# hellojialee/Improved-Body-Parts

Measured on NVIDIA H100. Metric: grouping images/sec @128x128 heatmaps, 30 persons/img, higher is better.
Workload: dtype f32 body-part maps, f32 keypoint maps; f64 coordinates/scores

## Files before the change

### improved_body_parts_b200/csrc/assemble.cuh

```cuda
#pragma once

#include "common.cuh"

namespace spg {

struct AssembleArgs {
    int n_images, image_base, use_bulk;
    double len_rate, connection_tole, min_mean_score;
    int remove_recon, min_parts;
    int refresh_len_check;
    unsigned long long *wire_flag;
    unsigned long long wire_flag_value;
    unsigned int *done_counter;
    Workspace ws;
};

constexpr int kAssembleThreads = 32;

struct alignas(16) RowRec {
    double total, maxlen;
    uint32_t mask;
    int cnt, birth, alive;
};
struct alignas(16) SlotRec {
// ... 449 lines not shown
            bulk_g2s(s_cij, ws.conn_ij + img_conn, (uint32_t)(LC * sizeof(uint32_t)), &bar);
        }
    } else {
        for (size_t i = lane; i < LC; i += 32) {
            s_cs[i] = ws.conn_score[img_conn + i];
            s_cn[i] = ws.conn_norm[img_conn + i];
            s_cij[i] = ws.conn_ij[img_conn + i];
        }
    }
    for (int k = lane; k < L; k += 32) s_cc[k] = ws.conn_count[(size_t)n * L + k];
    init_person_rows(t, ws, n, lane);
    stage_peaks(t, ws, n, lane, 32, nullptr);
    __syncwarp();
    if (a.use_bulk) mbar_wait(&bar, 0);
    const AsmResult res = assemble_limbs<false>(a, t, s_cs, s_cn, s_cij, s_cc, lane, nullptr);
    __syncthreads();
    emit_people(a, t, reinterpret_cast<double *>(smem_raw), assemble_conn_bytes(L, capP), s_out, n, img_in_call, res, lane, 32);
}

__global__ void __launch_bounds__(kAssembleThreads) assemble_kernel(AssembleArgs a) {
    extern __shared__ __align__(128) unsigned char smem_raw[];
    __shared__ uint64_t bar;
    __shared__ int s_out;
    if ((int)blockIdx.x >= a.n_images) return;
    assemble_image(a, smem_raw, bar, &s_out, a.image_base + blockIdx.x, blockIdx.x, threadIdx.x);
}

}
```

### improved_body_parts_b200/csrc/common.cuh

```cuda
#pragma once

#include <cuda_runtime.h>
#include <stdint.h>

#include <algorithm>

namespace spg {

#ifdef SPG_TRACE
constexpr int kTraceCtas = 64, kTraceSlots = 1024;
__device__ unsigned long long g_spg_trace[kTraceCtas * kTraceSlots];
__device__ __forceinline__ void trace_put(int slot, int dep, int mode) {
    if (blockIdx.x < kTraceCtas && (threadIdx.x & 31) == 0) {
        unsigned long long t;
        asm volatile("mov.u64 %0, %%clock64;" : "=l"(t) : "r"(dep) : "memory");
        unsigned long long *w = &g_spg_trace[blockIdx.x * kTraceSlots + slot];
        if (mode == 2) atomicCAS(w, 0ull, t);
        else if (mode == 3) atomicMax(w, t);
        else if (mode == 4) atomicAdd(w, (unsigned long long)(unsigned)dep);
        else *w = mode == 1 ? (unsigned long long)(unsigned)dep : t;
    }
}
#define SPG_TR(slot, dep) ::spg::trace_put((slot), (int)(dep), 0)
#define SPG_TRV(slot, v) ::spg::trace_put((slot), (int)(v), 1)
// ... 48 lines not shown
    int16_t out_from_part[kMaxOutJoints];
    double *peak_x, *peak_y;
    float *peak_score;
    uint32_t *peak_anchor;
    int32_t *peak_count;
    double *cand_prio, *cand_score;
    uint32_t *cand_ij;
    unsigned long long *cand_key;
    int32_t *cand_count;
    int32_t *surv_count;
    uint32_t *conn_ij;
    double *conn_score, *conn_norm;
    int32_t *conn_count;
    double *subset;
    int32_t *n_persons;
    double *people_xy;
    double *people_score;
    uint32_t *status;
    unsigned char *wire;
    long long wire_first;
    int wire_rows;
};

__device__ __forceinline__ uint32_t smem_u32(const void *p) { return (uint32_t)__cvta_generic_to_shared(p); }

__device__ __forceinline__ void mbar_init(uint64_t *bar, uint32_t count) {
    asm volatile("mbarrier.init.shared::cta.b64 [%0], %1;" ::"r"(smem_u32(bar)), "r"(count) : "memory");
}
__device__ __forceinline__ void fence_mbar_init() { asm volatile("fence.mbarrier_init.release.cluster;" ::: "memory"); }
__device__ __forceinline__ void fence_proxy_async() { asm volatile("fence.proxy.async.shared::cta;" ::: "memory"); }
__device__ __forceinline__ void mbar_expect_tx(uint64_t *bar, uint32_t bytes) {
    asm volatile("mbarrier.arrive.expect_tx.shared::cta.b64 _, [%0], %1;" ::"r"(smem_u32(bar)), "r"(bytes) : "memory");
}
__device__ __forceinline__ void bulk_g2s(void *dst_smem, const void *src_gmem, uint32_t bytes, uint64_t *bar) {
    asm volatile("cp.async.bulk.shared::cluster.global.mbarrier::complete_tx::bytes [%0], [%1], %2, [%3];" ::"r"(
                     smem_u32(dst_smem)),
                 "l"(src_gmem), "r"(bytes), "r"(smem_u32(bar))
                 : "memory");
}
__device__ __forceinline__ void mbar_arrive(uint64_t *bar) {
    asm volatile("mbarrier.arrive.shared::cta.b64 _, [%0];" ::"r"(smem_u32(bar)) : "memory");
}
__device__ __forceinline__ bool mbar_try_wait(uint64_t *bar, uint32_t parity) {
    uint32_t ok;
    asm volatile(
        "{\n"
// ... 50 lines not shown
```

### improved_body_parts_b200/csrc/group_unbounded.cuh

```cuda
#pragma once

#include <cub/cub.cuh>

#include "assemble.cuh"
#include "limb_score.cuh"
#include "nms_peaks.cuh"

namespace spg {

constexpr int kUbPeakThreads = 1024;
constexpr int kUbScoreThreads = 128;
constexpr int kUbAssembleThreads = 1024;
constexpr int kUbMaxPeaks = 65535;
constexpr int kUbMaxRows = 32767;

struct UbArgs {
    Workspace ws;
    const float *heat;
    const void *paf;
    int64_t heat_chan_stride, paf_chan_stride;
    int H, W;
    int32_t *row_count;
    const int64_t *row_off;
    const int64_t *seg_off;
    unsigned long long *cand_key_out;
    const uint32_t *sorted;
    uint32_t *cand_idx;
    unsigned char *used;
    PersonTable table;
};

template <bool WRITE>
__global__ void __launch_bounds__(kUbPeakThreads) ub_peaks_kernel(UbArgs u, NmsArgs a) {
    using Scan = cub::BlockScan<int, kUbPeakThreads>;
    __shared__ typename Scan::TempStorage scan_tmp;
    const int c = blockIdx.x, tid = threadIdx.x;
    const int H = u.H, W = u.W;
    const float *plane = u.heat + (int64_t)c * u.heat_chan_stride;
    const int64_t npix = (int64_t)H * W;
    int base = 0;
    for (int64_t p0 = 0; p0 < npix; p0 += kUbPeakThreads) {
        const int64_t p = p0 + tid;
        int y = 0, x = 0, pk = 0;
        if (p < npix) {
            y = (int)(p / W);
            x = (int)(p - (int64_t)y * W);
            pk = nms_is_peak(plane, 0, H, W, y, x, plane[p], a.thr) ? 1 : 0;
        }
        int pos, total;
        Scan(scan_tmp).ExclusiveSum(pk, pos, total);
        if (WRITE && pk) nms_finish_peak(a, plane, H, W, (size_t)c * u.ws.capP + base + pos, y, x);
        base += total;
        __syncthreads();
    }
    if (!WRITE && tid == 0) u.ws.peak_count[c] = base;
}

__device__ __forceinline__ unsigned long long ub_prio_key(double prio) {
    const unsigned long long b = (unsigned long long)__double_as_longlong(__dadd_rn(prio, 0.0));
    return (b >> 63) ? ~b : (b | 0x8000000000000000ull);
}

template <typename T, typename TA, bool WRITE>
__global__ void __launch_bounds__(kUbScoreThreads) ub_score_kernel(UbArgs u, ScoreArgs sa) {
    __shared__ double s_rcp[kScreenMaxMid + 1];
    for (int m = threadIdx.x; m <= kScreenMaxMid; m += blockDim.x) s_rcp[m] = m > 0 ? __ddiv_rn(1.0, (double)m) : 0.0;
    __syncthreads();
    const Workspace &ws = u.ws;
    const int k = blockIdx.x, i = blockIdx.y * kUbScoreThreads + threadIdx.x;
    const int pa = ws.limbs[2 * k], pb = ws.limbs[2 * k + 1];
    const int nA = ws.peak_count[pa], nB = ws.peak_count[pb];
    if (i >= nA || nB == 0) return;
    const int capP = ws.capP, H = u.H, W = u.W;
    const T *plane = reinterpret_cast<const T *>(u.paf) + (int64_t)k * u.paf_chan_stride;
    const PairGeom g{ws.peak_x + (size_t)pa * capP, ws.peak_y + (size_t)pa * capP, ws.peak_x + (size_t)pb * capP,
                     ws.peak_y + (size_t)pb * capP, ws.peak_score + (size_t)pa * capP, ws.peak_score + (size_t)pb * capP, s_rcp};
    const bool ain = inside_map(g.ax[i], g.ay[i], H, W);
    const TA thre2 = (TA)sa.thre2;
    const size_t slot = (size_t)k * capP + i;
    const int64_t out = WRITE ? u.row_off[slot] : 0;
    int nc = 0;
    bool bad = false;
    for (int j = 0; j < nB; j++) {
        double score, prio;
        const bool ok = score_pair_exact<T, 1, TA>(plane, H, W, sa, g, i, j, ain && inside_map(g.bx[j], g.by[j], H, W), thre2,
                                                   score, prio, bad);
        if (ok) {
            if (WRITE) {
                const int64_t o = out + nc;
                ws.cand_prio[o] = prio;
                ws.cand_score[o] = score;
                ws.cand_ij[o] = ((uint32_t)i << 16) | (uint32_t)j;
                ws.cand_key[o] = ub_prio_key(prio);
                u.cand_idx[o] = (uint32_t)o;
            }
            nc++;
        }
    }
    if (!WRITE) u.row_count[slot] = nc;
    if (bad) atomicOr(ws.status, kStSampleIndex);
}

__global__ void ub_match_kernel(UbArgs u) {
    const Workspace &ws = u.ws;
    const int k = blockIdx.x * blockDim.x + threadIdx.x;
    if (k >= ws.L) return;
    const int capP = ws.capP;
    const int pa = ws.limbs[2 * k], pb = ws.limbs[2 * k + 1];
    const int nA = ws.peak_count[pa], nB = ws.peak_count[pb];
    const int64_t c0 = u.seg_off[k], c1 = u.seg_off[k + 1];
    ws.cand_count[k] = (int)(c1 - c0);
    if (nA == 0 || nB == 0) {
        ws.conn_count[k] = -1;
        return;
    }
    unsigned char *usedA = u.used + (size_t)k * 2 * capP, *usedB = usedA + capP;
    const int lim = min(nA, nB);
    const size_t cb = (size_t)k * capP;
    int m = 0;
    for (int64_t c = c0; c < c1 && m < lim; c++) {
        const uint32_t idx = u.sorted[c];
        const uint32_t ij = ws.cand_ij[idx];
        const int i = (int)(ij >> 16), j = (int)(ij & 0xffff);
        if (usedA[i] || usedB[j]) continue;
        usedA[i] = 1;
        usedB[j] = 1;
        const double vx = __dsub_rn(ws.peak_x[(size_t)pb * capP + j], ws.peak_x[(size_t)pa * capP + i]);
        const double vy = __dsub_rn(ws.peak_y[(size_t)pb * capP + j], ws.peak_y[(size_t)pa * capP + i]);
        ws.conn_ij[cb + m] = ij;
        ws.conn_score[cb + m] = ws.cand_score[idx];
        ws.conn_norm[cb + m] = __dsqrt_rn(__dadd_rn(__dmul_rn(vx, vx), __dmul_rn(vy, vy)));
        m++;
    }
    ws.conn_count[k] = m;
}

__global__ void __launch_bounds__(kUbAssembleThreads) ub_assemble_kernel(UbArgs u, AssembleArgs a) {
    __shared__ int s_out;
    const Workspace &ws = a.ws;
    const PersonTable &t = u.table;
    const int tid = threadIdx.x, K = ws.K, L = ws.L, capP = ws.capP, capR = ws.capR;
    if (tid == 0) {
        int off = 0;
        for (int c = 0; c < K; c++) {
            t.off[c] = off;
            off += ws.peak_count[c];
        }
        t.off[K] = off;
    }
    for (int i = tid; i < K * capP; i += kUbAssembleThreads) {
        t.owner[i] = -1;
        t.ps[i] = ws.peak_score[i];
    }
    __syncthreads();
    int nrows = 0;
    if (tid == 0) {
        for (int k = 0; k < L; k++) {
            const int cc = ws.conn_count[k];
            if (cc < 0) continue;
            ConnCtx c;
// ... 41 lines not shown
```

### improved_body_parts_b200/csrc/limb_match.cuh

```cuda
#pragma once

#include "common.cuh"

namespace spg {

struct MatchArgs {
    int n_images, image_base, keys_valid;
    Workspace ws;
};

constexpr int kMatchThreads = 128;
constexpr int kMatchRegF64 = 16;
constexpr int kMatchRegCands = 16;

__device__ __forceinline__ bool key_better(double pa, int ia, double pb, int ib) {
    return pa > pb || (pa == pb && ia < ib);
}

__device__ __forceinline__ unsigned long long ordered_bits(double v) {
    const unsigned long long b = (unsigned long long)__double_as_longlong(v);
    return (b & 0x8000000000000000ull) ? ~b : (b | 0x8000000000000000ull);
}

template <int NS>
// ... 302 lines not shown
        case 5: case 6: m = match_rounds_ld<6>(sc, ws.capP, key8, nC, lane, 400 + 8 * k, ws.cand_score + cbase); break;
        default: m = match_rounds_ld<kMatchLdSlots>(sc, ws.capP, key8, nC, lane, 400 + 8 * k, ws.cand_score + cbase); break;
    }
    SPG_TR(400 + 8 * k + 5, m);
    if (coords_bar) mbar_wait(coords_bar, 0);
    for (int e = lane; e < m; e += 32) {
        const unsigned long long ke = sc.acc_key[e];
        const double score = ws.cand_score[cbase + sc.acc_cidx[e]];
        int rank = 0;
        for (int f = 0; f < m; f++) rank += sc.acc_key[f] > ke ? 1 : 0;
        const uint32_t ij = ~(uint32_t)ke;
        const int i = (int)(ij >> 16), j = (int)(ij & 0xffffu);
        const double vx = __dsub_rn(bx[j], ax[i]), vy = __dsub_rn(by[j], ay[i]);
        o_ij[rank] = ij;
        o_score[rank] = score;
        o_norm[rank] = __dsqrt_rn(__dadd_rn(__dmul_rn(vx, vx), __dmul_rn(vy, vy)));
    }
    __syncwarp();
    SPG_TR(400 + 8 * k + 6, m);
    return m;
}

__global__ void __launch_bounds__(kMatchThreads) limb_match_kernel(MatchArgs a) {
    const Workspace &ws = a.ws;
    const int lane = threadIdx.x & 31;
    const int w = (int)((blockIdx.x * (size_t)blockDim.x + threadIdx.x) >> 5);
    if (w >= a.n_images * ws.L) return;
    const int k = w % ws.L;
    const int n = a.image_base + w / ws.L;
    const size_t slot = (size_t)n * ws.L + k;
    const size_t obase = slot * ws.capP;
    const int m = match_limb(ws, n, k, lane, a.keys_valid != 0, ws.conn_ij + obase, ws.conn_score + obase, ws.conn_norm + obase);
    if (lane == 0) ws.conn_count[slot] = m;
}

}
```

### improved_body_parts_b200/csrc/limb_score.cuh

```cuda
#pragma once

#include "common.cuh"

namespace spg {

struct ScoreArgs {
    const void *paf;
    int64_t img_stride, chan_stride;
    int H, W, image_base, mid_num, screen;
    int crit1_strict;
    int exact_warps;
    double image_extent, thre2, connect_ration;
    Workspace ws;
};

constexpr int kScoreThreads = 512;
constexpr uint32_t kBulkChunkBytes = 32768;
constexpr int kScreenMaxMid = 63;
#ifndef SPG_SCREEN_SAMPLES
#define SPG_SCREEN_SAMPLES 10
#endif
constexpr int kScreenSamples = SPG_SCREEN_SAMPLES;
constexpr int kScreenMaxDim = 2048;
constexpr int kScreenSpreadFirst = kScreenSamples < 6 ? kScreenSamples : 6;
// ... 360 lines not shown
        while (lo < hi) {
            const int mid = (lo + hi + 1) >> 1;
            if ((int)s_prefix[mid] <= sidx) lo = mid; else hi = mid - 1;
        }
        const int bit = __fns(s_mask[lo], 0, sidx - (int)s_prefix[lo] + 1);
        const int p = (lo << 5) + bit;
        const int i = nB > 1 ? (int)__umulhi((uint32_t)p, magic) : p;
        const int j = p - i * nB;
        double score, prio;
        bool bad = false;
        const bool ok = score_pair_exact<T, 1, TA>(plane, H, W, a, g, i, j, s_ain[i] && s_bin[j], thre2_exact, score, prio, bad);
        if (bad) atomicOr(&s_flags, kStSampleIndex);
        if (ok) {
            const int pos = atomicAdd(&s_count, 1);
            if (pos < ws.capC) store_candidate<TA>(ws, out_base, pos, i, j, score, prio);
        }
    }
    __syncthreads();
    if (tid == 0) publish_limb(ws, n, slot, s_count, total_surv, s_flags);
}

template <typename T, bool STAGE, typename TA = T>
__global__ void __launch_bounds__(kScoreThreads, 3) limb_score_kernel(ScoreArgs a) {
    limb_score_plane<T, STAGE, TA>(a, a.ws, blockIdx.x / a.ws.L, blockIdx.x % a.ws.L);
}

struct ScoreImage {
    const void *paf;
    int64_t chan_stride;
    double image_extent;
    int H, W, slot;
};
constexpr int kScoreRaggedMaxImages = 128;
struct ScoreRagged {
    ScoreImage img[kScoreRaggedMaxImages];
};

template <typename T, bool STAGE, typename TA = T>
__global__ void __launch_bounds__(kScoreThreads, 3) limb_score_ragged_kernel(ScoreArgs a, const __grid_constant__ ScoreRagged r) {
    const ScoreImage &im = r.img[blockIdx.x / a.ws.L];
    ScoreArgs b = a;
    b.paf = im.paf;
    b.img_stride = 0;
    b.chan_stride = im.chan_stride;
    b.H = im.H;
    b.W = im.W;
    b.image_extent = im.image_extent;
    b.image_base = im.slot;
    limb_score_plane<T, STAGE, TA>(b, a.ws, 0, blockIdx.x % a.ws.L);
}

}
```

### improved_body_parts_b200/csrc/limb_score_persist.cuh

```cuda
#pragma once

#include "limb_score.cuh"

namespace spg {

constexpr int kPersistThreads = 1024;
constexpr int kPersistSlots = 3;
constexpr int kMetaSlots = 5;
constexpr int kWorkerWarps = kPersistThreads / 32 - 1;
constexpr int kPersistMaxCapP = 64;
constexpr int kScreenTailBypass = 4;
constexpr int kPersistListCap = 1024;

constexpr int kTrItemWords = 16, kTrItems = 64;
#define SPG_TR_ITEM(kind, j, f, dep) do { if ((j) < kTrItems) kind(kTrItemWords * (j) + (f), dep); } while (0)

struct PersistHdr {
    int nA, nB, npairs, n, k, special;
    uint32_t magic;
    int pad;
};

struct alignas(16) PeakSlot {
    double ax[kPersistMaxCapP], ay[kPersistMaxCapP], bx[kPersistMaxCapP], by[kPersistMaxCapP];
// ... 86 lines not shown
    const int H = a.H, W = a.W, capP = ws.capP, L = ws.L;
    const size_t plane_bytes = (size_t)H * W * sizeof(T);
    const size_t plane_stride = (plane_bytes + 127) & ~(size_t)127;
    double *s_rcp = reinterpret_cast<double *>(smem_raw);
    ScreenTab *s_tab = reinterpret_cast<ScreenTab *>(s_rcp + (kScreenMaxMid + 1));
    float *s_ts = reinterpret_cast<float *>(s_tab + (kScreenMaxMid + 1));
    MetaSlot *s_meta = reinterpret_cast<MetaSlot *>(smem_raw + screen_tables_bytes());
    unsigned char *s_planes = smem_raw + kPersistPlaneOffset;
    const int nE = min(max(a.exact_warps, 1), kWorkerWarps - 1), nS = kWorkerWarps - nE;

    if (tid == 0) {
        for (int s = 0; s < kPersistSlots; s++) {
            mbar_init(&bar_full[s], 2);
        }
        for (int e = 0; e < kMetaSlots; e++) {
            mbar_init(&bar_screened[e], nS);
            mbar_init(&bar_mfree[e], nE);
            s_meta[e].nsurv = 0; s_meta[e].ncand = 0; s_meta[e].bnext = 0; s_meta[e].flags = 0;
        }
        s_bias_bytes = 4u * kScreenBias * (uint32_t)(W + 1);
        fence_mbar_init();
    }
    if (tid >= 32 && tid < 32 + kScreenMaxMid + 1) build_screen_row(a, tid - 32, s_rcp, s_tab, s_ts, true);
    __syncthreads();

    const bool screen = a.screen && a.mid_num <= kScreenMaxMid && H <= kScreenMaxDim && W <= kScreenMaxDim;
    const T thre2 = sizeof(TA) == 8 ? f32_not_above(a.thre2) : (T)a.thre2;
    const TA thre2_exact = (TA)a.thre2;
    auto plane_of = [&](int n_local, int k) {
        return reinterpret_cast<const T *>(a.paf) + (int64_t)n_local * a.img_stride + (int64_t)k * a.chan_stride;
    };

    if (warp == 0) {
        constexpr int kMaxE = kPersistMaxCapP / 32;
        double r_xa[kMaxE], r_ya[kMaxE], r_xb[kMaxE], r_yb[kMaxE];
        float r_sa[kMaxE], r_sb[kMaxE];
        int r_cntA = 0, r_cntB = 0, r_item = 0;
        auto fetch = [&]() {
            int t = 0;
            if (lane == 0) t = (int)atomicAdd(queue, 1u);
            r_item = __shfl_sync(0xffffffffu, t, 0);
            const int item = min(r_item, n_items - 1);
            const int n_local = item / L, k = item - n_local * L;
            const int n = a.image_base + n_local;
            const int pa = ws.limbs[2 * k], pb = ws.limbs[2 * k + 1];
            r_cntA = ws.peak_count[(size_t)n * ws.K + pa];
            r_cntB = ws.peak_count[(size_t)n * ws.K + pb];
// ... 184 lines not shown
```

### improved_body_parts_b200/csrc/match_assemble.cuh

```cuda
#pragma once

#include "assemble.cuh"
#include "limb_match.cuh"

namespace spg {

constexpr int kMAMatchWarps = 7;
constexpr int kMAThreads = 32 * (1 + kMAMatchWarps);
constexpr int kMAMaxThreads = 512;

inline size_t match_assemble_smem_bytes(int K, int L, int capP, int capR, int n_match) {
    return assemble_conn_bytes(L, capP) + assemble_smem_bytes(K, capP, capR) + 2 * (size_t)K * capP * sizeof(double) +
           (size_t)n_match * match_scratch_bytes(capP);
}

__global__ void __launch_bounds__(kMAMaxThreads) match_assemble_kernel(AssembleArgs a, int keys_valid) {
    extern __shared__ __align__(128) unsigned char smem_raw[];
    __shared__ int s_ready[kMaxLimbs];
    __shared__ AsmResult s_res;
    __shared__ int s_out;
    __shared__ uint64_t s_bar;
    const Workspace &ws = a.ws;
    if ((int)blockIdx.x >= a.n_images) return;
    const int n = a.image_base + blockIdx.x;
    const int tid = threadIdx.x, lane = tid & 31, warp = tid >> 5;
    const int K = ws.K, L = ws.L, capP = ws.capP, capR = ws.capR;
    SPG_TR(warp == 0 ? 0 : 2 + warp, 0);
    const size_t LC = (size_t)L * capP;
    double *s_cs = reinterpret_cast<double *>(smem_raw);
    double *s_cn = s_cs + LC;
    uint32_t *s_cij = reinterpret_cast<uint32_t *>(s_cn + LC);
    int *s_cc = reinterpret_cast<int *>(s_cij + LC);
    unsigned char *table_base = smem_raw + assemble_conn_bytes(L, capP);
    PersonTable t = make_person_table(table_base, K, capP, capR);
    double *s_xy = reinterpret_cast<double *>(table_base + assemble_smem_bytes(K, capP, capR));
    t.px = s_xy;
    t.py = s_xy + (size_t)K * capP;
    const int n_match = (int)blockDim.x / 32 - 1;
    if (tid < L) s_ready[tid] = 0;
    const bool bulk = a.use_bulk != 0;
    if (tid == 0 && bulk) {
        mbar_init(&s_bar, 1);
        fence_mbar_init();
    }
    __syncthreads();
    if (tid == 0 && bulk) {
        const size_t KP = (size_t)K * capP, g = (size_t)n * KP;
        mbar_expect_tx(&s_bar, (uint32_t)(KP * (sizeof(float) + 2 * sizeof(double))));
        bulk_g2s(t.ps, ws.peak_score + g, (uint32_t)(KP * sizeof(float)), &s_bar);
        bulk_g2s(s_xy, ws.peak_x + g, (uint32_t)(KP * sizeof(double)), &s_bar);
        bulk_g2s(s_xy + KP, ws.peak_y + g, (uint32_t)(KP * sizeof(double)), &s_bar);
    }
    if (warp == 0) {
        SPG_TR(1, 0);
        init_person_rows(t, ws, n, lane);
        __syncwarp();
        if (bulk) mbar_wait(&s_bar, 0);
        const AsmResult res = assemble_limbs<true>(a, t, s_cs, s_cn, s_cij, s_cc, lane, s_ready);
        if (lane == 0) s_res = res;
    } else {
        if (!bulk) {
            stage_peaks(t, ws, n, tid - 32, 32 * n_match, s_xy);
            asm volatile("bar.sync 1, %0;" ::"r"(32 * n_match) : "memory");
        }
        unsigned char *scratch = reinterpret_cast<unsigned char *>(s_xy + 2 * (size_t)K * capP) + (size_t)(warp - 1) * match_scratch_bytes(capP);
        for (int k = warp - 1; k < L; k += n_match) {
            uint32_t *o_ij = s_cij + (size_t)k * capP;
// ... 28 lines not shown
```

### improved_body_parts_b200/csrc/nms_peaks.cuh

```cuda
#pragma once

#include "common.cuh"

namespace spg {

struct NmsArgs {
    const float *heat;
    int64_t img_stride, chan_stride;
    int H, W, band_rows, radius, use_bulk, image_base;
    float thr;
    Workspace ws;
};

constexpr int kNmsThreads = 256;
constexpr int kNmsBufs = 3;

__device__ __forceinline__ bool nms_is_peak(const float *buf, int lo, int H, int W, int y, int x, float v, float thr) {
    if (!(v >= thr) || v == 0.0f) return false;
#pragma unroll
    for (int dy = -1; dy <= 1; dy++) {
        const int yy = y + dy;
        if (yy < 0 || yy >= H) continue;
        const float *row = buf + (size_t)(yy - lo) * W;
#pragma unroll
// ... 162 lines not shown

    const Workspace &ws = a.ws;
    const int tid = threadIdx.x;
    const int n = a.image_base + n_local;
    const int H = a.H, W = a.W, br = a.band_rows;
    const float *plane = a.heat + (int64_t)n_local * a.img_stride + (int64_t)c * a.chan_stride;

    const int nb = (H + br - 1) / br;
    const size_t band_floats = nb == 1 ? (size_t)H * W : (size_t)(br + 2) * W;
    const size_t buf_stride = (band_floats + 31) & ~(size_t)31;
    const int nbufs = min(nb, kNmsBufs);
    float *buf0 = reinterpret_cast<float *>(smem_raw);
    uint32_t *s_list = reinterpret_cast<uint32_t *>(buf0 + (size_t)nbufs * buf_stride);
    uint32_t *s_sorted = s_list + ws.capP;
    uint16_t *s_queue = reinterpret_cast<uint16_t *>(s_sorted + ws.capP);

    if (tid == 0) {
        s_count = 0;
        if (a.use_bulk) {
            for (int i = 0; i < kNmsBufs; i++) mbar_init(&bar[i], 1);
            fence_mbar_init();
        }
    }
    __syncthreads();

    auto band_lo = [&](int b) { return max(b * br - 1, 0); };
    auto band_hi = [&](int b) { return min((b + 1) * br + 1, H); };
    auto issue = [&](int b) {
        const int lo = band_lo(b), hi = band_hi(b);
        const uint32_t bytes = (uint32_t)(hi - lo) * W * sizeof(float);
        mbar_expect_tx(&bar[b % kNmsBufs], bytes);
        bulk_g2s(buf0 + (size_t)(b % kNmsBufs) * buf_stride, plane + (size_t)lo * W, bytes, &bar[b % kNmsBufs]);
    };

    if (a.use_bulk && tid == 0)
        for (int b = 0; b < nbufs; b++) issue(b);

    for (int b = 0; b < nb; b++) {
        float *buf = a.use_bulk ? buf0 + (size_t)(b % kNmsBufs) * buf_stride : buf0;
        const int lo = band_lo(b), hi = band_hi(b);
        if (a.use_bulk) {
            mbar_wait(&bar[b % kNmsBufs], (b / kNmsBufs) & 1);
        } else {
            const int cnt = (hi - lo) * W;
            for (int i = tid; i < cnt; i += kNmsThreads) buf[i] = plane[(size_t)lo * W + i];
            __syncthreads();
// ... 99 lines not shown
```

### improved_body_parts_b200/csrc/nms_peaks_banded.cuh

```cuda
#pragma once

#include "nms_peaks_persist.cuh"

namespace spg {

constexpr int kNmsBMaxSlots = 16;
constexpr int kNmsBTeams = 4;
constexpr int kNmsBBandGroups = 1024;

struct NmsBanding {
    int band_rows, n_bands, slots, teams;
    size_t band_stride, smem;
};
inline NmsBanding nms_banding(int H, int W, int capP, size_t smem_limit) {
    NmsBanding g{};
    const int W4 = W / 4;
    const size_t fixed = kNmsPLists * (size_t)capP * sizeof(uint32_t) + (size_t)kNmsPScanners * 32 * kNmsPMaxIter * sizeof(uint16_t) + 64;
    if (smem_limit <= fixed) return g;
    g.teams = kNmsBTeams;
    const int team_warps = kNmsPScanners / kNmsBTeams;
    g.band_rows = std::max(1, std::min(H, kNmsBBandGroups / std::max(W4, 1)));
    if ((size_t)g.band_rows * W4 > (size_t)team_warps * 32 * kNmsPMaxIter) return g;
    g.n_bands = (H + g.band_rows - 1) / g.band_rows;
    g.band_stride = (((size_t)std::min(g.band_rows + 2, H) * W * sizeof(float)) + 127) & ~(size_t)127;
// ... 10 lines not shown
    const Workspace &ws = a.ws;
    const int tid = threadIdx.x, lane = tid & 31, warp = tid >> 5;
    const int H = a.H, W = a.W, K = ws.K, capP = ws.capP;
    const int BR = a.band_rows, S = n_slots, NB = n_bands;
    constexpr int T = kNmsBTeams, TW = kNmsPScanners / kNmsBTeams;
    const size_t band_stride = (((size_t)min(BR + 2, H) * W * sizeof(float)) + 127) & ~(size_t)127;
    uint32_t *s_lists = reinterpret_cast<uint32_t *>(smem_raw + (size_t)S * band_stride);
    uint16_t *s_queues = reinterpret_cast<uint16_t *>(s_lists + kNmsPLists * (size_t)capP);
    const int W4 = W >> 2;
    const uint32_t w4_magic = W4 > 1 ? 0xffffffffu / (uint32_t)W4 + 1u : 0u;

    if (tid == 0) {
        for (int s = 0; s < S; s++) {
            mbar_init(&bar_full[s], 1);
            mbar_init(&bar_free[s], TW);
        }
        for (int l = 0; l < kNmsPLists; l++) {
            mbar_init(&bar_ready[l], kNmsPScanners);
            mbar_init(&bar_lfree[l], 1);
            s_cnt[l] = 0;
        }
        fence_mbar_init();
    }
    __syncthreads();

    const int G = gridDim.x;
    const int nj = ((int)blockIdx.x < n_items) ? (n_items - 1 - (int)blockIdx.x) / G + 1 : 0;

    if (warp == 0) {
        if (lane == 0) {
            int s = 0, round = 0;
            for (int j = 0; j < nj; j++) {
                const int item = (int)blockIdx.x + j * G;
                const int n_local = item / K, c = item - n_local * K;
                const float *plane = a.heat + (int64_t)n_local * a.img_stride + (int64_t)c * a.chan_stride;
                for (int b = 0; b < NB; b++) {
                    if (round > 0) mbar_wait_sleep(&bar_free[s], (round - 1) & 1);
                    const int r0 = b * BR, lo = max(r0 - 1, 0), hi = min(r0 + BR + 1, H);
                    const uint32_t bytes = (uint32_t)((size_t)(hi - lo) * W * sizeof(float));
                    mbar_expect_tx(&bar_full[s], bytes);
                    bulk_g2s(smem_raw + (size_t)s * band_stride, plane + (size_t)lo * W, bytes, &bar_full[s]);
                    if (++s == S) { s = 0; round++; }
                }
            }
        }
    } else if (warp <= kNmsPScanners) {
// ... 43 lines not shown
```

### improved_body_parts_b200/csrc/nms_peaks_persist.cuh

```cuda
#pragma once

#include "nms_peaks.cuh"

namespace spg {

constexpr int kNmsPSlots = 3;

constexpr int kNmsTrWords = 16, kNmsTrPlanes = 64;
#define SPG_NMS_TR(kind, j, f, dep) do { if ((j) < kNmsTrPlanes) kind(kNmsTrWords * (j) + (f), dep); } while (0)

inline size_t nms_persist_smem_bytes(int H, int W, int capP) {
    const size_t plane = (((size_t)H * W * sizeof(float)) + 127) & ~(size_t)127;
    const size_t queues = (size_t)kNmsPScanners * 32 * kNmsPMaxIter * sizeof(uint16_t);
    return kNmsPSlots * plane + kNmsPLists * (size_t)capP * sizeof(uint32_t) + queues + 64;
}

template <int R>
__global__ void __launch_bounds__(kNmsPThreads, 1) nms_peaks_persist_kernel(NmsArgs a, int n_items) {
    extern __shared__ __align__(128) unsigned char smem_raw[];
    __shared__ uint64_t bar_full[kNmsPSlots], bar_free[kNmsPSlots], bar_ready[kNmsPLists], bar_lfree[kNmsPLists];
    __shared__ int s_cnt[kNmsPLists];

    const Workspace &ws = a.ws;
    const int tid = threadIdx.x, lane = tid & 31, warp = tid >> 5;
    const int H = a.H, W = a.W, K = ws.K, capP = ws.capP;
    const size_t plane_bytes = (size_t)H * W * sizeof(float);
    const size_t plane_stride = (plane_bytes + 127) & ~(size_t)127;
    uint32_t *s_lists = reinterpret_cast<uint32_t *>(smem_raw + kNmsPSlots * plane_stride);
    uint16_t *s_queues = reinterpret_cast<uint16_t *>(s_lists + kNmsPLists * (size_t)capP);
    const int W4 = W >> 2, groups = H * W4;
    const uint32_t w4_magic = W4 > 1 ? 0xffffffffu / (uint32_t)W4 + 1u : 0u;

    if (tid == 0) {
        for (int s = 0; s < kNmsPSlots; s++) {
            mbar_init(&bar_full[s], 1);
            mbar_init(&bar_free[s], 1);
        }
        for (int l = 0; l < kNmsPLists; l++) {
            mbar_init(&bar_ready[l], kNmsPScanners);
            mbar_init(&bar_lfree[l], 1);
            s_cnt[l] = 0;
        }
        fence_mbar_init();
    }
    __syncthreads();

    const int G = gridDim.x;
    const int nj = ((int)blockIdx.x < n_items) ? (n_items - 1 - (int)blockIdx.x) / G + 1 : 0;

    if (warp == 0) {
        if (lane == 0) {
            for (int j = 0; j < nj; j++) {
                const int s = j % kNmsPSlots;
                SPG_NMS_TR(SPG_TR, j, 0, j);
                if (j >= kNmsPSlots) mbar_wait_sleep(&bar_free[s], ((j / kNmsPSlots) - 1) & 1);
                const int item = (int)blockIdx.x + j * G;
                const int n_local = item / K, c = item - n_local * K;
                const unsigned char *src =
                    reinterpret_cast<const unsigned char *>(a.heat + (int64_t)n_local * a.img_stride + (int64_t)c * a.chan_stride);
                unsigned char *dst = smem_raw + s * plane_stride;
                mbar_expect_tx(&bar_full[s], (uint32_t)plane_bytes);
                for (size_t off = 0; off < plane_bytes; off += 32768) {
                    const uint32_t bytes = (uint32_t)min((size_t)32768, plane_bytes - off);
                    bulk_g2s(dst + off, src + off, bytes, &bar_full[s]);
                }
                SPG_NMS_TR(SPG_TR, j, 1, j);
            }
// ... 53 lines not shown
```

### improved_body_parts_b200/csrc/postnet.cuh

```cuda
#pragma once

#include <cuda_fp16.h>

#include "common.cuh"

namespace spg {

constexpr int kPostThreads = 256;
constexpr int kPostTW = 64, kPostTH = 32;
constexpr int kPostC1 = 96, kPostR1 = 48;
constexpr int kPostCS = 32, kPostRS = 20;
constexpr int kMaxNetChannels = 64;

constexpr int kPostMaxScales = 4;
struct PostScale {
    const void *net;
    int net_is_f16;
    long long img_stride, pair_stride, chan_stride;
    int h, w;
    int crop_h, crop_w;
    double sx2, sy2;
};

struct PostArgs {
// ... 26 lines not shown
    c[2] = __fadd_rn(__fmul_rn(__fmul_rn(__fsub_rn(__fmul_rn(a2, y), a3), y), y), 1.0f);
    c[3] = __fsub_rn(__fsub_rn(__fsub_rn(1.0f, c[0]), c[1]), c[2]);
}

__device__ __forceinline__ int axis_entry(int d, double scale, float c[4]) {
    const float f = (float)__dsub_rn(__dmul_rn(__dadd_rn((double)d, 0.5), scale), 0.5);
    const float fl = floorf(f);
    cubic_coeffs(__fsub_rn(f, fl), c);
    return (int)fl - 1;
}

__device__ __forceinline__ float tap4(float a0, float a1, float a2, float a3, const float *c) {
    return __fadd_rn(__fadd_rn(__fadd_rn(__fmul_rn(a0, c[0]), __fmul_rn(a1, c[1])), __fmul_rn(a2, c[2])), __fmul_rn(a3, c[3]));
}

__device__ __forceinline__ int clampi(int v, int lo, int hi) { return min(max(v, lo), hi); }

struct AxisTab {
    int s;
    float c[4];
};

__global__ void __launch_bounds__(kPostThreads) postnet_generic_kernel(PostArgs a) {
    __shared__ AxisTab t2x[kPostTW], t2y[kPostTH], t1x[kPostC1], t1y[kPostR1];
    __shared__ float s0[kPostRS * kPostCS];
    __shared__ float s1[kPostRS * kPostC1];
    __shared__ float s2[kPostR1 * kPostC1];
    __shared__ float s3[kPostR1 * kPostTW];
    __shared__ int r_lo[4];

    const int tid = threadIdx.x;
    const int tile = blockIdx.x, c = blockIdx.y, n = blockIdx.z;
    const int ty = tile / a.tiles_x, tx = tile - ty * a.tiles_x;
    const int ox0 = tx * a.tile_w, oy0 = ty * a.tile_h;
    const int tw = min(a.tile_w, a.W - ox0), th = min(a.tile_h, a.H - oy0);
    const PostScale &S = a.sc[0];
    const bool identity = S.crop_h == a.H && S.crop_w == a.W;

    if (tid < tw) t2x[tid].s = axis_entry(ox0 + tid, S.sx2, t2x[tid].c);
    if (tid >= 64 && tid < 64 + th) t2y[tid - 64].s = axis_entry(oy0 + tid - 64, S.sy2, t2y[tid - 64].c);
    __syncthreads();
    if (tid == 0) {
        const int c_lo = identity ? ox0 : clampi(t2x[0].s, 0, S.crop_w - 1), c_hi = identity ? ox0 + tw - 1 : clampi(t2x[tw - 1].s + 3, 0, S.crop_w - 1);
        const int rr_lo = identity ? oy0 : clampi(t2y[0].s, 0, S.crop_h - 1), rr_hi = identity ? oy0 + th - 1 : clampi(t2y[th - 1].s + 3, 0, S.crop_h - 1);
        r_lo[0] = c_lo; r_lo[1] = c_hi - c_lo + 1;
        r_lo[2] = rr_lo; r_lo[3] = rr_hi - rr_lo + 1;
// ... 468 lines not shown
            const PostScale &S = im.sc[t];
            const bool identity = IDENT || (S.crop_h == im.H && S.crop_w == im.W);
            const PostRange R = post_range(T);
            const float4 W[4] = {T.wph[0], T.wph[1], T.wph[2], T.wph[3]};
            post_commit(s0, pv0, pv1, R, warp, lane);
            __syncthreads();
            {
                int tn = t + 1, cn = c;
                if (tn == a.n_fused) { tn = 0; cn = c + 1; }
                if (cn < c_end) post_prefetch<F16>(pv0, pv1, im.sc[tn], TT[tn], a, n, cn, warp, lane);
            }
            post_x4_passes(T, R, W, s0, s1, s2, tid, lane, warp);
            post_resize2_h<IDENT>(T, s2, s3, identity, tw, th, lane, warp);
            post_resize2_v<SINGLE, IDENT>(acc, T, s2, s3, identity, a, im, out, ox0, oy0, tw, th, 4 * R.q_lo, 4 * R.p_lo,
                                          a.scale_index == 0 && t == 0, nf, nf_rcp, nf_small, lane, warp);
            __syncthreads();
        }
        post_store_acc<SINGLE>(acc, im, out, tw, th, lane, warp);
    }
}

template <bool SINGLE, bool IDENT, bool F16>
__global__ void __launch_bounds__(kPostThreads, 2) postnet_kernel(PostArgs a) {
    postnet_tile<SINGLE, IDENT, F16>(a, a, blockIdx.x, blockIdx.y, blockIdx.z);
}

constexpr int kPostR_R1 = 64;
constexpr size_t postR_smem_bytes() {
    return sizeof(PostTabs) + sizeof(float) * ((size_t)kPostF_RS * kPostF_CS + (size_t)kPostF_RS * kPostF_C1 +
                                               (size_t)kPostF_R1 * kPostF_C1 + (size_t)kPostR_R1 * kPostF_C1);
}
static_assert(kPostR_R1 * kPostTW <= kPostF_RS * (kPostF_CS + kPostF_C1), "pass 3's output fits where the source tile was");

template <int CS, typename T, typename Val>
__device__ __forceinline__ float warp_linear(int xs, int ys, int w, int h, const T *g, int pitch, int x0, int y0, const Val &val) {
    const int xf = xs >> 5, yf = ys >> 5;
    const int sx = clampi(xf >> 5, -32768, 32767), sy = clampi(yf >> 5, -32768, 32767);
    const float fx = __fmul_rn((float)(xf & 31), 0.03125f), fy = __fmul_rn((float)(yf & 31), 0.03125f);
    const float gx = __fsub_rn(1.0f, fx), gy = __fsub_rn(1.0f, fy);
    const bool x0in = sx >= 0 && sx < w, x1in = sx + 1 >= 0 && sx + 1 < w;
    const bool y0in = sy >= 0 && sy < h, y1in = sy + 1 >= 0 && sy + 1 < h;
    const T *u = g + (sy - y0) * pitch + (sx - x0) * CS;
    const float t00 = (y0in && x0in) ? val(u[0]) : 0.0f, t01 = (y0in && x1in) ? val(u[CS]) : 0.0f;
    const float t10 = (y1in && x0in) ? val(u[pitch]) : 0.0f, t11 = (y1in && x1in) ? val(u[pitch + CS]) : 0.0f;
    return __fadd_rn(__fadd_rn(__fadd_rn(__fmul_rn(t00, __fmul_rn(gy, gx)), __fmul_rn(t01, __fmul_rn(gy, fx))),
                               __fmul_rn(t10, __fmul_rn(fy, gx))), __fmul_rn(t11, __fmul_rn(fy, fx)));
// ... 63 lines not shown
        const PostOut out = post_out(a, im, n, c, ox0, oy0, more_follow);
        double acc[SINGLE ? 1 : kPostKY][SINGLE ? 1 : kPostKX];
        post_load_acc<SINGLE>(acc, a, im, c, out.pbase, tw, th, lane, warp);
        post_commit(s0, pv0, pv1, R, warp, lane);
        __syncthreads();
        if (c + 1 < c_end) post_prefetch<F16>(pv0, pv1, S, T, a, n, c + 1, warp, lane);
        post_x4_passes(T, R, W, s0, s1, su, tid, lane, warp);
        for (int e = tid; e < R1 * C1; e += kPostThreads) {
            const int Y = e / C1, X = e - Y * C1;
            sr[Y * kPostF_C1 + X] = warp_linear<1>(rowX[Y] + colA[X], rowY[Y] + colB[X], Wp, Hp, su, kPostF_C1, bx0, by0,
                                                   [](float v) { return v; });
        }
        __syncthreads();
        post_resize2_h<false>(T, sr, s3, identity, tw, th, lane, warp);
        post_resize2_v<SINGLE, false>(acc, T, sr, s3, identity, a, im, out, ox0, oy0, tw, th, c_lo, y_lo, a.scale_index == 0, nf,
                                      nf_rcp, nf_small, lane, warp);
        __syncthreads();
        post_store_acc<SINGLE>(acc, im, out, tw, th, lane, warp);
    }
}

template <bool SINGLE, bool F16>
__global__ void __launch_bounds__(kPostThreads, 2) postnet_rot_kernel(PostArgs a) {
    postnet_rot_tile<SINGLE, F16>(a, a, blockIdx.x, blockIdx.y, blockIdx.z);
}

constexpr int kPostI_TW = 128, kPostI_TH = 32;
constexpr int kPostI_Q = kPostI_TW / 4, kPostI_P = kPostI_TH / 4;
constexpr int kPostI_RS = kPostI_P + 4, kPostI_CS = kPostI_Q + 4;
constexpr int kPostI_S0 = kPostI_CS;
constexpr int kPostI_LD = (kPostI_RS * kPostI_CS + kPostThreads - 1) / kPostThreads;

template <bool F16, class I>
__device__ __forceinline__ void postnet_x4_ident_tile(const PostArgs &a, const I &im, int tile, int chunk, int n) {
    __shared__ float s0[2][kPostI_RS * kPostI_S0];
    __shared__ __align__(16) float s1[2][kPostI_RS * kPostI_TW];
    __shared__ int s_o1x[kPostI_Q + 1][5], s_o1y[kPostI_P][5];
    __shared__ float4 s_wph[4];

    const int tid = threadIdx.x;
    const PostScale &S = im.sc[0];
    const int c_begin = chunk * a.chan_chunk, c_end = min(c_begin + a.chan_chunk, a.n_out);
    const int ty = tile / im.tiles_x, tx = tile - ty * im.tiles_x;
    const int ox0 = tx * kPostI_TW, oy0 = ty * kPostI_TH;
    const int tw = min(kPostI_TW, im.W - ox0), th = min(kPostI_TH, im.H - oy0);
    const int q_lo = ox0 >> 2, Q = ((ox0 + tw - 1) >> 2) - q_lo + 1, p_lo = oy0 >> 2, P = ((oy0 + th - 1) >> 2) - p_lo + 1;
// ... 138 lines not shown
                } else {
#pragma unroll
                    for (int k = 0; k < 4; k++) {
                        if (4 * p2 + k < th) {
                            const float e[4] = {r[k].x, r[k].y, r[k].z, r[k].w};
#pragma unroll
                            for (int x = 0; x < 4; x++)
                                if (4 * x2 + x < tw) od[(size_t)k * im.W + x] = (double)e[x];
                        }
                    }
                }
            }
        }
        if (c + 1 < c_end) {
            commit(buf ^ 1);
            if (c + 2 < c_end) prefetch(c + 2);
        }
        __syncthreads();
    }
}

template <bool F16>
__global__ void __launch_bounds__(kPostThreads, 4) postnet_x4_ident_kernel(PostArgs a) {
    postnet_x4_ident_tile<F16>(a, a, blockIdx.x, blockIdx.y, blockIdx.z);
}

constexpr int kPostRaggedMaxImages = 64;
struct PostRagged {
    int n;
    PostImage img[kPostRaggedMaxImages];
};

template <class R>
__device__ __forceinline__ const auto &post_ragged_image(const R &r, int cta) {
    int lo = 0, hi = r.n - 1;
    while (lo < hi) {
        const int mid = (lo + hi + 1) >> 1;
        if (r.img[mid].first_cta <= cta) lo = mid;
        else hi = mid - 1;
    }
    return r.img[lo];
}

template <bool F16>
__global__ void __launch_bounds__(kPostThreads, 4) postnet_x4_ident_ragged_kernel(PostArgs a, const __grid_constant__ PostRagged r) {
    const PostImage &im = post_ragged_image(r, blockIdx.x);
    postnet_x4_ident_tile<F16>(a, im, blockIdx.x - im.first_cta, blockIdx.y, 0);
}

template <bool F16>
__global__ void __launch_bounds__(kPostThreads, 2) postnet_ragged_kernel(PostArgs a, const __grid_constant__ PostRagged r) {
    const PostImage &im = post_ragged_image(r, blockIdx.x);
    postnet_tile<true, false, F16>(a, im, blockIdx.x - im.first_cta, blockIdx.y, 0);
}

constexpr int kPostParamBytes = 32764;
constexpr int kPostItemsMaxImages = (int)((kPostParamBytes - sizeof(PostArgs) - 8) / sizeof(PostItemsImage));
struct PostItemsRagged {
    int n;
    PostItemsImage img[kPostItemsMaxImages];
};
static_assert(sizeof(PostArgs) + sizeof(PostItemsRagged) <= kPostParamBytes, "a launch's parameters fit the kernel-parameter limit");

template <bool IDENT, bool F16>
__global__ void __launch_bounds__(kPostThreads, 2) postnet_items_ragged_kernel(PostArgs a, const __grid_constant__ PostItemsRagged r) {
    const PostItemsImage &im = post_ragged_image(r, blockIdx.x);
    postnet_tile<false, IDENT, F16>(a, im, blockIdx.x - im.first_cta, blockIdx.y, 0);
}

template <bool SINGLE, bool F16>
__global__ void __launch_bounds__(kPostThreads, 2) postnet_rot_ragged_kernel(PostArgs a, const __grid_constant__ PostItemsRagged r) {
    const PostItemsImage &im = post_ragged_image(r, blockIdx.x);
    postnet_rot_tile<SINGLE, F16>(a, im, blockIdx.x - im.first_cta, blockIdx.y, 0);
}

}
```

### improved_body_parts_b200/csrc/prenet.cuh

```cuda
#pragma once

#include "postnet.cuh"

namespace spg {

constexpr int kPreThreads = 128;
constexpr int kPreLanes = 8;

struct PreArgs {
    const unsigned char *src;
    long long img_stride, row_stride;
    int h, w;
    int H1, W1;
    int Hp, Wp;
    int copy;
    int n_body;
    int pad_value;
    double scale;
    unsigned char *grid;
    float *out;
    long long out_stride;
    double rot[6];
};

// ... 30 lines not shown
#pragma unroll
        for (int ch = 0; ch < 3; ch++)
            S[r][ch] = row[col[0] + ch] * ax[0] + row[col[1] + ch] * ax[1] + row[col[2] + ch] * ax[2] + row[col[3] + ch] * ax[3];
    }
    float b[4];
#pragma unroll
    for (int k = 0; k < 4; k++) b[k] = __fmul_rn((float)by[k], 2.384185791015625e-07f);
#pragma unroll
    for (int ch = 0; ch < 3; ch++) {
        if (3 * x + ch < a.n_body) {
            float t = __fmul_rn((float)S[3][ch], b[3]);
            t = __fadd_rn(__fmul_rn((float)S[2][ch], b[2]), t);
            t = __fadd_rn(__fmul_rn((float)S[1][ch], b[1]), t);
            t = __fadd_rn(__fmul_rn((float)S[0][ch], b[0]), t);
            v[ch] = clampi(__float2int_rn(t), 0, 255);
        } else {
            const int acc = S[0][ch] * by[0] + S[1][ch] * by[1] + S[2][ch] * by[2] + S[3][ch] * by[3];
            v[ch] = clampi((acc + (1 << 21)) >> 22, 0, 255);
        }
    }
}

__global__ void __launch_bounds__(kPreThreads) prenet_resize_kernel(PreArgs a) {
    const int x = blockIdx.x * kPreThreads + threadIdx.x, y = blockIdx.y, n = blockIdx.z;
    if (x >= a.Wp) return;
    int v[3];
    prenet_pixel(a, a.src + n * a.img_stride, y, x, v);
    unsigned char *g = a.grid + (((long long)n * a.Hp + y) * a.Wp + x) * 3;
    g[0] = (unsigned char)v[0]; g[1] = (unsigned char)v[1]; g[2] = (unsigned char)v[2];
}

template <bool ROT>
__global__ void __launch_bounds__(kPreThreads) prenet_kernel(PreArgs a) {
    __shared__ float lut[256];
    prenet_lut(lut);
    const int x = blockIdx.x * kPreThreads + threadIdx.x, y = blockIdx.y, n = blockIdx.z;
    if (x >= a.Wp) return;
    float f[3];
    if (ROT) {
        const double xd = (double)x, yd = (double)y;
        const int xs = __double2int_rn(__dmul_rn(__dmul_rn(a.rot[0], xd), 1024.0)) +
                       __double2int_rn(__dmul_rn(__dadd_rn(__dmul_rn(a.rot[1], yd), a.rot[2]), 1024.0)) + 16;
        const int ys = __double2int_rn(__dmul_rn(__dmul_rn(a.rot[3], xd), 1024.0)) +
                       __double2int_rn(__dmul_rn(__dadd_rn(__dmul_rn(a.rot[4], yd), a.rot[5]), 1024.0)) + 16;
        const unsigned char *g = a.grid + (long long)n * a.Hp * a.Wp * 3;
#pragma unroll
        for (int ch = 0; ch < 3; ch++)
            f[ch] = warp_linear<3>(xs, ys, a.Wp, a.Hp, g + ch, 3 * a.Wp, 0, 0, [&](unsigned char v) { return lut[v]; });
    } else {
        int v[3];
        prenet_pixel(a, a.src + n * a.img_stride, y, x, v);
        f[0] = lut[v[0]]; f[1] = lut[v[1]]; f[2] = lut[v[2]];
    }
    float *o = a.out + n * a.out_stride + ((long long)y * a.Wp + x) * 3;
    float *m = a.out + n * a.out_stride + ((long long)(a.Hp + y) * a.Wp + (a.Wp - 1 - x)) * 3;
    o[0] = f[0]; o[1] = f[1]; o[2] = f[2];
// ... 5 lines not shown
```

### improved_body_parts_b200/csrc/spgroup.cu

```cuda
#include "../../include/spgroup.h"

#include <cuda_runtime.h>

#include <algorithm>
#include <cmath>
#include <cstdarg>
#include <cstdio>
#include <cstdlib>
#include <cstring>
#include <new>
#include <string>
#include <vector>

#include "assemble.cuh"
#include "common.cuh"
#include "group_unbounded.cuh"
#include "limb_match.cuh"
#include "limb_score.cuh"
#include "limb_score_persist.cuh"
#include "match_assemble.cuh"
#include "nms_peaks.cuh"
#include "nms_peaks_persist.cuh"
#include "nms_peaks_banded.cuh"
#include "postnet.cuh"
// ... 76 lines not shown
        if (prev != dev) cudaSetDevice(dev);
    }
    ~DeviceGuard() {
        int cur = -1;
        cudaGetDevice(&cur);
        if (prev >= 0 && cur != prev) cudaSetDevice(prev);
    }
};

int grow(spg_handle *h, Scratch &s, size_t bytes) {
    if (s.bytes >= bytes) return SPG_OK;
    if (s.p) cudaFree(s.p);
    s.p = nullptr;
    s.bytes = 0;
    SPG_CUDA(h, cudaMalloc(&s.p, bytes));
    s.bytes = bytes;
    return SPG_OK;
}

template <typename... P, typename... A>
int launch(spg_handle *h, int stage, const char *name, void (*kern)(P...), dim3 grid, int block, size_t smem, cudaStream_t st,
           const A &...args) {
    if (smem > 0) SPG_CUDA(h, cudaFuncSetAttribute(kern, cudaFuncAttributeMaxDynamicSharedMemorySize, (int)smem));
    kern<<<grid, block, smem, st>>>(args...);
    h->stage_kernel[stage] = name;
    h->launches++;
    SPG_CUDA(h, cudaGetLastError());
    return SPG_OK;
}

int check_batch(spg_handle *h, int n) {
    if (n < 0 || n > h->cfg.max_batch) return fail(h, SPG_E_INVALID, "n_images %d outside [0, max_batch=%d]", n, h->cfg.max_batch);
    return SPG_OK;
}

int check_dims(spg_handle *h, int n, int H, int W) {
    int rc;
    if ((rc = check_batch(h, n))) return rc;
    if (H < 2 || W < 2 || H > h->cfg.max_h || W > h->cfg.max_w || H > 32767 || W > 32767)
        return fail(h, SPG_E_INVALID, "map %dx%d outside [2, %dx%d]", H, W, h->cfg.max_h, h->cfg.max_w);
    return SPG_OK;
}

int check_params(spg_handle *h, const spg_params *p) {
    if (!p) return fail(h, SPG_E_INVALID, "params is NULL");
    if (p->offset_radius < 0 || p->offset_radius > kMaxRefineRadius)
        return fail(h, SPG_E_INVALID, "offset_radius %d outside [0, %d]", p->offset_radius, kMaxRefineRadius);
    if (p->mid_num < 1) return fail(h, SPG_E_INVALID, "mid_num must be >= 1");
    return SPG_OK;
}
// ... 1553 lines not shown
```

Baseline: 660,600.

## Enable programmatic dependent launch across all pipeline kernels

Launches every kernel with the programmatic stream serialization attribute through cudaLaunchKernelEx. Each kernel calls griddepcontrol.wait followed by launch_dependents at entry, after any mbarrier or table setup where possible, so the next kernel's launch and prologue can overlap the tail of the previous one. The persistent score kernel swaps a full __syncthreads for a named barrier so the producer warp can arrive without blocking. This targets launch latency between many small back-to-back kernels, at the cost of triggering dependents early, which keeps extra CTAs resident while they wait.

Result: no change. 664,700 (median of 6 runs) (+0.6%).

```diff
diff --git a/improved_body_parts_b200/csrc/assemble.cuh b/improved_body_parts_b200/csrc/assemble.cuh
--- a/improved_body_parts_b200/csrc/assemble.cuh
+++ b/improved_body_parts_b200/csrc/assemble.cuh
@@ -495,6 +495,7 @@
     extern __shared__ __align__(128) unsigned char smem_raw[];
     __shared__ uint64_t bar;
     __shared__ int s_out;
+    grid_dep_enter();
     if ((int)blockIdx.x >= a.n_images) return;
     assemble_image(a, smem_raw, bar, &s_out, a.image_base + blockIdx.x, blockIdx.x, threadIdx.x);
 }
diff --git a/improved_body_parts_b200/csrc/common.cuh b/improved_body_parts_b200/csrc/common.cuh
--- a/improved_body_parts_b200/csrc/common.cuh
+++ b/improved_body_parts_b200/csrc/common.cuh
@@ -94,6 +94,13 @@
     int wire_rows;
 };
 
+__device__ __forceinline__ void grid_dep_wait() { asm volatile("griddepcontrol.wait;" ::: "memory"); }
+__device__ __forceinline__ void grid_dep_trigger() { asm volatile("griddepcontrol.launch_dependents;" ::: "memory"); }
+__device__ __forceinline__ void grid_dep_enter() {
+    grid_dep_wait();
+    grid_dep_trigger();
+}
+
 __device__ __forceinline__ uint32_t smem_u32(const void *p) { return (uint32_t)__cvta_generic_to_shared(p); }
 
 __device__ __forceinline__ void mbar_init(uint64_t *bar, uint32_t count) {
diff --git a/improved_body_parts_b200/csrc/group_unbounded.cuh b/improved_body_parts_b200/csrc/group_unbounded.cuh
--- a/improved_body_parts_b200/csrc/group_unbounded.cuh
+++ b/improved_body_parts_b200/csrc/group_unbounded.cuh
@@ -32,6 +32,7 @@
 
 template <bool WRITE>
 __global__ void __launch_bounds__(kUbPeakThreads) ub_peaks_kernel(UbArgs u, NmsArgs a) {
+    grid_dep_enter();
     using Scan = cub::BlockScan<int, kUbPeakThreads>;
     __shared__ typename Scan::TempStorage scan_tmp;
     const int c = blockIdx.x, tid = threadIdx.x;
@@ -63,6 +64,7 @@
 
 template <typename T, typename TA, bool WRITE>
 __global__ void __launch_bounds__(kUbScoreThreads) ub_score_kernel(UbArgs u, ScoreArgs sa) {
+    grid_dep_enter();
     __shared__ double s_rcp[kScreenMaxMid + 1];
     for (int m = threadIdx.x; m <= kScreenMaxMid; m += blockDim.x) s_rcp[m] = m > 0 ? __ddiv_rn(1.0, (double)m) : 0.0;
     __syncthreads();
@@ -102,6 +104,7 @@
 }
 
 __global__ void ub_match_kernel(UbArgs u) {
+    grid_dep_enter();
     const Workspace &ws = u.ws;
     const int k = blockIdx.x * blockDim.x + threadIdx.x;
     if (k >= ws.L) return;
@@ -136,6 +139,7 @@
 }
 
 __global__ void __launch_bounds__(kUbAssembleThreads) ub_assemble_kernel(UbArgs u, AssembleArgs a) {
+    grid_dep_enter();
     __shared__ int s_out;
     const Workspace &ws = a.ws;
     const PersonTable &t = u.table;
diff --git a/improved_body_parts_b200/csrc/limb_match.cuh b/improved_body_parts_b200/csrc/limb_match.cuh
--- a/improved_body_parts_b200/csrc/limb_match.cuh
+++ b/improved_body_parts_b200/csrc/limb_match.cuh
@@ -348,6 +348,7 @@
 }
 
 __global__ void __launch_bounds__(kMatchThreads) limb_match_kernel(MatchArgs a) {
+    grid_dep_enter();
     const Workspace &ws = a.ws;
     const int lane = threadIdx.x & 31;
     const int w = (int)((blockIdx.x * (size_t)blockDim.x + threadIdx.x) >> 5);
diff --git a/improved_body_parts_b200/csrc/limb_score.cuh b/improved_body_parts_b200/csrc/limb_score.cuh
--- a/improved_body_parts_b200/csrc/limb_score.cuh
+++ b/improved_body_parts_b200/csrc/limb_score.cuh
@@ -406,6 +406,7 @@
 
 template <typename T, bool STAGE, typename TA = T>
 __global__ void __launch_bounds__(kScoreThreads, 3) limb_score_kernel(ScoreArgs a) {
+    grid_dep_enter();
     limb_score_plane<T, STAGE, TA>(a, a.ws, blockIdx.x / a.ws.L, blockIdx.x % a.ws.L);
 }
 
@@ -422,6 +423,7 @@
 
 template <typename T, bool STAGE, typename TA = T>
 __global__ void __launch_bounds__(kScoreThreads, 3) limb_score_ragged_kernel(ScoreArgs a, const __grid_constant__ ScoreRagged r) {
+    grid_dep_enter();
     const ScoreImage &im = r.img[blockIdx.x / a.ws.L];
     ScoreArgs b = a;
     b.paf = im.paf;
diff --git a/improved_body_parts_b200/csrc/limb_score_persist.cuh b/improved_body_parts_b200/csrc/limb_score_persist.cuh
--- a/improved_body_parts_b200/csrc/limb_score_persist.cuh
+++ b/improved_body_parts_b200/csrc/limb_score_persist.cuh
@@ -132,7 +132,13 @@
         fence_mbar_init();
     }
     if (tid >= 32 && tid < 32 + kScreenMaxMid + 1) build_screen_row(a, tid - 32, s_rcp, s_tab, s_ts, true);
-    __syncthreads();
+    grid_dep_enter();
+    if (warp == 0) {
+        asm volatile("bar.arrive 1, %0;" ::"r"(kPersistThreads) : "memory");
+        __syncwarp();
+    } else {
+        asm volatile("bar.sync 1, %0;" ::"r"(kPersistThreads) : "memory");
+    }
 
     const bool screen = a.screen && a.mid_num <= kScreenMaxMid && H <= kScreenMaxDim && W <= kScreenMaxDim;
     const T thre2 = sizeof(TA) == 8 ? f32_not_above(a.thre2) : (T)a.thre2;
diff --git a/improved_body_parts_b200/csrc/match_assemble.cuh b/improved_body_parts_b200/csrc/match_assemble.cuh
--- a/improved_body_parts_b200/csrc/match_assemble.cuh
+++ b/improved_body_parts_b200/csrc/match_assemble.cuh
@@ -43,6 +43,7 @@
         mbar_init(&s_bar, 1);
         fence_mbar_init();
     }
+    grid_dep_enter();
     __syncthreads();
     if (tid == 0 && bulk) {
         const size_t KP = (size_t)K * capP, g = (size_t)n * KP;
diff --git a/improved_body_parts_b200/csrc/nms_peaks.cuh b/improved_body_parts_b200/csrc/nms_peaks.cuh
--- a/improved_body_parts_b200/csrc/nms_peaks.cuh
+++ b/improved_body_parts_b200/csrc/nms_peaks.cuh
@@ -208,6 +208,7 @@
             fence_mbar_init();
         }
     }
+    grid_dep_enter();
     __syncthreads();
 
     auto band_lo = [&](int b) { return max(b * br - 1, 0); };
diff --git a/improved_body_parts_b200/csrc/nms_peaks_banded.cuh b/improved_body_parts_b200/csrc/nms_peaks_banded.cuh
--- a/improved_body_parts_b200/csrc/nms_peaks_banded.cuh
+++ b/improved_body_parts_b200/csrc/nms_peaks_banded.cuh
@@ -56,6 +56,7 @@
         }
         fence_mbar_init();
     }
+    grid_dep_enter();
     __syncthreads();
 
     const int G = gridDim.x;
diff --git a/improved_body_parts_b200/csrc/nms_peaks_persist.cuh b/improved_body_parts_b200/csrc/nms_peaks_persist.cuh
--- a/improved_body_parts_b200/csrc/nms_peaks_persist.cuh
+++ b/improved_body_parts_b200/csrc/nms_peaks_persist.cuh
@@ -43,6 +43,7 @@
         }
         fence_mbar_init();
     }
+    grid_dep_enter();
     __syncthreads();
 
     const int G = gridDim.x;
diff --git a/improved_body_parts_b200/csrc/postnet.cuh b/improved_body_parts_b200/csrc/postnet.cuh
--- a/improved_body_parts_b200/csrc/postnet.cuh
+++ b/improved_body_parts_b200/csrc/postnet.cuh
@@ -72,6 +72,7 @@
 };
 
 __global__ void __launch_bounds__(kPostThreads) postnet_generic_kernel(PostArgs a) {
+    grid_dep_enter();
     __shared__ AxisTab t2x[kPostTW], t2y[kPostTH], t1x[kPostC1], t1y[kPostR1];
     __shared__ float s0[kPostRS * kPostCS];
     __shared__ float s1[kPostRS * kPostC1];
@@ -586,6 +587,7 @@
 
 template <bool SINGLE, bool IDENT, bool F16>
 __global__ void __launch_bounds__(kPostThreads, 2) postnet_kernel(PostArgs a) {
+    grid_dep_enter();
     postnet_tile<SINGLE, IDENT, F16>(a, a, blockIdx.x, blockIdx.y, blockIdx.z);
 }
 
@@ -695,6 +697,7 @@
 
 template <bool SINGLE, bool F16>
 __global__ void __launch_bounds__(kPostThreads, 2) postnet_rot_kernel(PostArgs a) {
+    grid_dep_enter();
     postnet_rot_tile<SINGLE, F16>(a, a, blockIdx.x, blockIdx.y, blockIdx.z);
 }
 
@@ -879,6 +882,7 @@
 
 template <bool F16>
 __global__ void __launch_bounds__(kPostThreads, 4) postnet_x4_ident_kernel(PostArgs a) {
+    grid_dep_enter();
     postnet_x4_ident_tile<F16>(a, a, blockIdx.x, blockIdx.y, blockIdx.z);
 }
 
@@ -901,12 +905,14 @@
 
 template <bool F16>
 __global__ void __launch_bounds__(kPostThreads, 4) postnet_x4_ident_ragged_kernel(PostArgs a, const __grid_constant__ PostRagged r) {
+    grid_dep_enter();
     const PostImage &im = post_ragged_image(r, blockIdx.x);
     postnet_x4_ident_tile<F16>(a, im, blockIdx.x - im.first_cta, blockIdx.y, 0);
 }
 
 template <bool F16>
 __global__ void __launch_bounds__(kPostThreads, 2) postnet_ragged_kernel(PostArgs a, const __grid_constant__ PostRagged r) {
+    grid_dep_enter();
     const PostImage &im = post_ragged_image(r, blockIdx.x);
     postnet_tile<true, false, F16>(a, im, blockIdx.x - im.first_cta, blockIdx.y, 0);
 }
@@ -921,12 +927,14 @@
 
 template <bool IDENT, bool F16>
 __global__ void __launch_bounds__(kPostThreads, 2) postnet_items_ragged_kernel(PostArgs a, const __grid_constant__ PostItemsRagged r) {
+    grid_dep_enter();
     const PostItemsImage &im = post_ragged_image(r, blockIdx.x);
     postnet_tile<false, IDENT, F16>(a, im, blockIdx.x - im.first_cta, blockIdx.y, 0);
 }
 
 template <bool SINGLE, bool F16>
 __global__ void __launch_bounds__(kPostThreads, 2) postnet_rot_ragged_kernel(PostArgs a, const __grid_constant__ PostItemsRagged r) {
+    grid_dep_enter();
     const PostItemsImage &im = post_ragged_image(r, blockIdx.x);
     postnet_rot_tile<SINGLE, F16>(a, im, blockIdx.x - im.first_cta, blockIdx.y, 0);
 }
diff --git a/improved_body_parts_b200/csrc/prenet.cuh b/improved_body_parts_b200/csrc/prenet.cuh
--- a/improved_body_parts_b200/csrc/prenet.cuh
+++ b/improved_body_parts_b200/csrc/prenet.cuh
@@ -76,6 +76,7 @@
 }
 
 __global__ void __launch_bounds__(kPreThreads) prenet_resize_kernel(PreArgs a) {
+    grid_dep_enter();
     const int x = blockIdx.x * kPreThreads + threadIdx.x, y = blockIdx.y, n = blockIdx.z;
     if (x >= a.Wp) return;
     int v[3];
@@ -86,6 +87,7 @@
 
 template <bool ROT>
 __global__ void __launch_bounds__(kPreThreads) prenet_kernel(PreArgs a) {
+    grid_dep_enter();
     __shared__ float lut[256];
     prenet_lut(lut);
     const int x = blockIdx.x * kPreThreads + threadIdx.x, y = blockIdx.y, n = blockIdx.z;
diff --git a/improved_body_parts_b200/csrc/spgroup.cu b/improved_body_parts_b200/csrc/spgroup.cu
--- a/improved_body_parts_b200/csrc/spgroup.cu
+++ b/improved_body_parts_b200/csrc/spgroup.cu
@@ -122,10 +122,23 @@
 int launch(spg_handle *h, int stage, const char *name, void (*kern)(P...), dim3 grid, int block, size_t smem, cudaStream_t st,
            const A &...args) {
     if (smem > 0) SPG_CUDA(h, cudaFuncSetAttribute(kern, cudaFuncAttributeMaxDynamicSharedMemorySize, (int)smem));
-    kern<<<grid, block, smem, st>>>(args...);
+    cudaLaunchAttribute attr[1];
+    attr[0].id = cudaLaunchAttributeProgrammaticStreamSerialization;
+    attr[0].val.programmaticStreamSerializationAllowed = 1;
+    cudaLaunchConfig_t cfg{};
+    cfg.gridDim = grid;
+    cfg.blockDim = dim3((unsigned)block);
+    cfg.dynamicSmemBytes = smem;
+    cfg.stream = st;
+    cfg.attrs = attr;
+    cfg.numAttrs = 1;
+    const cudaError_t e = cudaLaunchKernelEx(&cfg, kern, args...);
     h->stage_kernel[stage] = name;
     h->launches++;
-    SPG_CUDA(h, cudaGetLastError());
+    if (e != cudaSuccess) {
+        cudaGetLastError();
+        return fail(h, SPG_E_CUDA, "launch of %s failed: %s", name, cudaGetErrorString(e));
+    }
     return SPG_OK;
 }
 
```
